# szpajder/dumphfdl

Measured on AMD Instinct MI355X. Metric: wideband I/Q Msamples/s (cf32 ingest -> decoded HFDL PDUs) at fixed channel count, higher is better.
Workload: dtype f32

## Files before the change

dumphfdl_amd/csrc/fft_kernels.hip:

```cpp
#include <hip/hip_ext.h>
#include "kernels.h"
#include "retune_launch.h"
#include "fft_core.h"
#include "fft_regs.h"

namespace hfdl {

template <int FMT>
__device__ __forceinline__ float2 load_sample(const void *__restrict__ raw, int i)
{
	if (FMT == SFMT_CS16) {
		const short2 v = ((const short2 *)raw)[i];
		return make_float2((float)v.x / 32767.5f, (float)v.y / 32767.5f);
	} else if (FMT == SFMT_CU8) {
		const uchar2 v = ((const uchar2 *)raw)[i];
		return make_float2(((float)v.x - 63.5f) / 127.0f, ((float)v.y - 63.5f) / 127.0f);
	}
	return ((const float2 *)raw)[i];
}

__device__ __forceinline__ void store_out(float2 *out, const FftOutLayout &lay, unsigned i, size_t at, float2 v)
{
	if (lay.kind == TAPL_PLAIN) { out[at] = v; return; }
	float *o = (float *)out + tap_index_f(lay.kind, 1 << lay.row_log, (size_t)(2 * lay.row_stride), lay.chan, (int)(i >> lay.row_log), (int)(i & ((1u << lay.row_log) - 1u)), 0);
	o[0] = v.x;
	o[4] = v.y;
}

template <int FMT>
__global__ __launch_bounds__(FFT_THREADS) void fft_pass1(const float2 *__restrict__ hist, FftInputs in,
		int split, float2 *__restrict__ hist_next, float2 *__restrict__ out, FftPlan p, NcoJob job, int riders)
{
	if ((int)blockIdx.x < riders) { if (blockIdx.y == 0) nco_table_segment(job, (int)blockIdx.x * FFT_THREADS + (int)threadIdx.x); return; }
	const int bid = (int)blockIdx.x - riders;
	const int rx = (int)blockIdx.y;
	const void *__restrict__ fresh = in.fresh[rx];
	if (hist != nullptr) hist += rx * in.hist_stride;
	if (hist_next != nullptr) hist_next += rx * in.hist_stride;
	out += (size_t)rx * (size_t)p.n;
	extern __shared__ float2 sm[];
	const int cs = p.n >> p.l1;
	const int c0 = bid * FFT_TILE;
	const int total = p.r1 * FFT_TILE;
	for (int e = threadIdx.x; e < total; e += FFT_THREADS) {
		const int r = e >> FFT_TILE_LOG, col = e & (FFT_TILE - 1);
		const int c = c0 + col;
		float2 v = make_float2(0.f, 0.f);
		if (c < cs) {
			const int idx = r * cs + c;
			v = idx < split ? hist[idx] : load_sample<FMT>(fresh, idx - split);
			if (hist_next != nullptr && idx >= p.n - split) hist_next[idx - (p.n - split)] = v;
		}
		sm[e] = v;
	}
	float2 *ltw = sm + total;
	for (int t = threadIdx.x; t < p.r1; t += FFT_THREADS) ltw[t] = p.tw1[t];
	__syncthreads();
	lds_fft_columns<-1>(sm, p.r1, p.l1, FFT_TILE, FFT_TILE_LOG, ltw);
	for (int e = threadIdx.x; e < total; e += FFT_THREADS) {
		const int k1 = e >> FFT_TILE_LOG, col = e & (FFT_TILE - 1);
		const int c = c0 + col;
		if (c >= cs) continue;
		float2 v = sm[bitrev(k1, p.l1) * FFT_TILE + col];
		const unsigned ex = ((unsigned)k1 * (unsigned)c) & (unsigned)(p.n - 1);
		out[(size_t)k1 * cs + c] = cmul(v, unit_twiddle(ex, p.logn));
	}
}

__global__ __launch_bounds__(FFT_THREADS) void fft_pass2(float2 *__restrict__ buf, FftPlan p, NcoJob job, int riders)
{
	if ((int)blockIdx.x < riders) { if (blockIdx.y == 0) nco_table_segment(job, (int)blockIdx.x * FFT_THREADS + (int)threadIdx.x); return; }
	const int bid = (int)blockIdx.x - riders;
	buf += (size_t)blockIdx.y * (size_t)p.n;
	extern __shared__ float2 sm[];
	const int r23 = p.n >> p.l1, ncol = p.r1 * p.r3;
	const int cc0 = bid * FFT_TILE;
	const int total = p.r2 * FFT_TILE;
	for (int e = threadIdx.x; e < total; e += FFT_THREADS) {
		const int r = e >> FFT_TILE_LOG, col = e & (FFT_TILE - 1);
		const int cc = cc0 + col;
		float2 v = make_float2(0.f, 0.f);
		if (cc < ncol) {
			const int k1 = cc >> p.l3, n3 = cc & (p.r3 - 1);
			v = buf[(size_t)k1 * r23 + (size_t)r * p.r3 + n3];
		}
// ... 169 lines not shown
			}
		}
		if (AHEAD) {
#pragma unroll
			for (int n1 = 0; n1 < 16; n1++) x[n1] = xn[n1];
		}
	}
}

template <int B>
__global__ __launch_bounds__(16 * B) void fft_rpass3(const float2 *__restrict__ in, float2 *__restrict__ out, FftPlan p, int shifted,
		FftOutLayout lay, NcoJob job, int riders, int tpw, int64_t out_rx_stride)
{
	constexpr int NT = 16 * B, R = 16 * B;
	if ((int)blockIdx.x < riders) { if (blockIdx.y == 0) nco_table_segment(job, (int)blockIdx.x * NT + (int)threadIdx.x); return; }
	in += (size_t)blockIdx.y * (size_t)p.n;
	out += blockIdx.y * out_rx_stride;
	__shared__ float2 ex[B * FR_PITCH];
	__shared__ float2 ltw[16 * B];
	const int bid = ((int)blockIdx.x - riders) * tpw, tid = (int)threadIdx.x;
	const int r23 = p.n >> p.l1;
	const int col = tid & 15, n2 = tid >> 4;
	float2 pre[16], pn[16];
	auto load = [&](float2 (&v)[16], int tile) {
		const int cc0 = tile * 16;
		const float2 *src = in + (size_t)(cc0 >> p.l1) * R + (size_t)(cc0 & (p.r1 - 1)) * r23;
#pragma unroll
		for (int i = 0; i < 16; i++) {
			const int e = tid + i * NT;
			v[i] = src[(size_t)(e / R) * r23 + (e % R)];
		}
	};
	load(pre, bid);
	ltw[tid] = p.tw3[tid];
	const unsigned half = shifted ? (unsigned)(p.n >> 1) : 0u;
	for (int t = 0; t < tpw; t++) {
		const int tile = bid + t;
		const int k2g = (tile * 16) >> p.l1, k10 = (tile * 16) & (p.r1 - 1);
		__syncthreads();
#pragma unroll
		for (int i = 0; i < 16; i++) {
			const int e = tid + i * NT, tcol = e / R, n3 = e % R;
			ex[n3 * 16 + ((tcol + n3) & 15)] = pre[i];
		}
		if (t + 1 < tpw) load(pn, tile + 1);
		__syncthreads();
		float2 x[16];
#pragma unroll
		for (int n1 = 0; n1 < 16; n1++) {
			const int r = n2 + B * n1;
			x[n1] = ex[r * 16 + ((col + r) & 15)];
		}
		__syncthreads();
		stage_a(x, ex, ltw, n2, col);
		__syncthreads();
#pragma unroll
		for (int i = 0; i < 256 / NT; i++) {
			const int tt = tid + i * NT, tcol = tt & 15, ka = tt >> 4;
			float2 z[B];
			stage_b<B>(z, ex, ka, tcol);
			const unsigned kbase = (unsigned)(k10 + tcol) + ((unsigned)k2g << p.l1);
#pragma unroll
			for (int kb = 0; kb < B; kb++) {
				const unsigned k = kbase + ((unsigned)(ka + 16 * kb) << (p.l1 + p.l2));
				const unsigned i2 = (k + half) & (unsigned)(p.n - 1);
				const size_t at = lay.row_log ? (size_t)(i2 >> lay.row_log) * (size_t)lay.row_stride + (i2 & ((1u << lay.row_log) - 1u)) : (size_t)i2;
				store_out(out, lay, i2, at, z[slot_small<B>(kb)]);
			}
		}
#pragma unroll
		for (int i = 0; i < 16; i++) pre[i] = pn[i];
	}
}

static void launch_rpass(const void *kernel, dim3 grid, int logr, hipStream_t st, hipEvent_t start, hipEvent_t stop, void **args)
{
	(void)hipExtLaunchKernel(kernel, grid, dim3(1u << logr), args, 0, st, start, stop, 0);
}
template <int B> static const void *rpass1_of(int fmt)
{
	return fmt == SFMT_CS16 ? (const void *)fft_rpass1<B, SFMT_CS16, false> : fmt == SFMT_CU8 ? (const void *)fft_rpass1<B, SFMT_CU8, false> : (const void *)fft_rpass1<B, SFMT_CF32, false>;
}

__global__ void retune_channelizer_kernel(ChanConst *cc, NcoState *chain, float2 *cont, int c, ChanConst k)
{
	if (blockIdx.x != 0 || threadIdx.x != 0) return;
	cc[c] = k;
	chain[c] = NcoState{ 0, 0.f, 0, 0 };
	cont[c] = make_float2(0.f, 0.f);
}

void launch_retune_channelizer(ChanConst *cc, NcoState *chain, float2 *cont, int c, const ChanConst &k, hipStream_t st, hipEvent_t done)
{
	hipExtLaunchKernelGGL(retune_channelizer_kernel, dim3(1), dim3(64), 0, st, nullptr, done, 0, cc, chain, cont, c, k);
}

static bool fast_plan(const FftPlan &p) { return p.l1 >= 6 && p.l1 <= 8 && p.l2 >= 6 && p.l2 <= 8 && p.l3 >= 6 && p.l3 <= 8; }

__global__ __launch_bounds__(256) void mixed_copy_kernel(float2 *__restrict__ plain, float *__restrict__ taps, const float2 *__restrict__ block,
		int dir, int l1, int l2, int l3, int q, int m, size_t rs_f, int slot)
{
	const size_t n = (size_t)1 << (l1 + l2 + l3);
	for (size_t e = (size_t)blockIdx.x * 256 + threadIdx.x; e < n; e += (size_t)gridDim.x * 256) {
		const int ka = (int)(e & 15), n3 = (int)(e >> 4) & ((1 << l3) - 1), kb = (int)(e >> (4 + l3)) & ((1 << (l2 - 4)) - 1), k1 = (int)(e >> (l2 + l3));
		const int k2 = ka + 16 * kb, jp = mixed_bin(natural_bin_of(k1, k2, q, l1), l1);
		float2 *pl = plain + ((size_t)k1 << (l2 + l3)) + ((size_t)k2 << l3) + n3;
		if (dir == 2) {
			*pl = block[((size_t)(jp >> 4) << (l2 - q + l3 + 4)) + (size_t)mixed_row(k2, n3, q, l3) * 16 + (jp & 15)];
			continue;
		}
		float *t = taps + tap_index_f(TAPL_OCTET, m, rs_f, slot, mixed_tap_row(k2, n3, q, l3), jp, 0);
		const float r3 = (float)(1 << l3), ir3 = 1.0f / r3;
		if (dir == 0) { const float2 v = *pl; t[0] = v.x * r3; t[4] = v.y * r3; }
		else *pl = make_float2(t[0] * ir3, t[4] * ir3);
	}
}

static void launch_mixed_copy(const FftPlan &p, const Geometry &g, float2 *plain, float *taps, const float2 *block, int dir, int slot, hipStream_t st)
{
	hipLaunchKernelGGL(mixed_copy_kernel, dim3(2048), dim3(256), 0, st, plain, taps, block, dir, p.l1, p.l2, p.l3, g.mix_q, g.m, (size_t)g.tap_row_stride * 2, slot);
}
void launch_mixed_tap_pack(const FftPlan &p, const Geometry &g, const float2 *plain, float2 *taps, int slot, hipStream_t st) { launch_mixed_copy(p, g, (float2 *)plain, (float *)taps, nullptr, 0, slot, st); }
void launch_mixed_tap_unpack(const FftPlan &p, const Geometry &g, const float2 *taps, int slot, float2 *plain, hipStream_t st) { launch_mixed_copy(p, g, plain, (float *)taps, nullptr, 1, slot, st); }
void launch_mixed_block_unpack(const FftPlan &p, const Geometry &g, const float2 *slot, float2 *plain, hipStream_t st) { launch_mixed_copy(p, g, plain, nullptr, slot, 2, 0, st); }

void launch_fft_forward(const FftPlan &p, const float2 *hist, const FftInputs &in, int fmt, int split, float2 *hist_next,
		float2 *work, float2 *out, bool shifted, hipStream_t st, FftOutLayout lay, hipEvent_t done, NcoJob nco, hipEvent_t input_read, hipEvent_t start, FftVariant var)
{
	const unsigned nrx = (unsigned)in.nrx;
	const int64_t ors = in.out_stride;
	const int c1 = (p.n >> p.l1), c2 = p.r1 * p.r3, c3 = p.r1 * p.r2;
	const int g1 = (c1 + FFT_TILE - 1) / FFT_TILE, g2 = (c2 + FFT_TILE - 1) / FFT_TILE, g3 = (c3 + FFT_TILE - 1) / FFT_TILE;
	nco.nseg = 3;
	if (fast_plan(p)) {
		const bool mix = var.mix_out != nullptr, run1 = var.passes & 1, run2 = var.passes & 2, run3 = var.passes & 4;
		if (mix) nco.nseg = 2;
		auto riders_of = [&](int l) { const int nt = 1 << l; return nco.cc ? (nco.nch + nt - 1) / nt : 0; };
		const int rd1 = riders_of(p.l1), rd2 = riders_of(p.l2), rd3 = mix ? 0 : riders_of(p.l3);
		auto tpw_of = [](int tiles) { return tiles % 4 == 0 && tiles >= 4096 ? 4 : tiles % 2 == 0 && tiles >= 1024 ? 2 : 1; };
		const int t3 = tpw_of(g3);
		FftPlan plan = p;
		FftInputs inputs = in;
		int tpw = 1, shift = shifted ? 1 : 0, keep = mix && run3 ? 1 : 0;
		int64_t out_stride = ors;
		nco.seg = 0;
		if (run1) {
			void *args[] = { &hist, &inputs, &split, &hist_next, &work, &plan, &nco, (void *)&rd1, &tpw };
			launch_rpass(p.l1 == 6 ? rpass1_of<4>(fmt) : p.l1 == 7 ? rpass1_of<8>(fmt) : rpass1_of<16>(fmt), dim3(g1 + rd1, nrx), p.l1, st, start, input_read, args);
		}
		nco.seg = 1;
		if (run2) {
			void *args[] = { &work, &plan, &nco, (void *)&rd2, &tpw, &var.mix_out, &var.mix_q, &keep, &var.mix_rx_stride };
			launch_rpass(p.l2 == 6 ? (const void *)fft_rpass2<4, false> : p.l2 == 7 ? (const void *)fft_rpass2<8, false> : (const void *)fft_rpass2<16, false>,
					dim3(g2 + rd2, nrx), p.l2, st, nullptr, mix || !run3 ? done : nullptr, args);
		}
		nco.seg = 2;
		if (run3) {
			void *args[] = { &work, &out, &plan, &shift, &lay, &nco, (void *)&rd3, (void *)&t3, &out_stride };
			launch_rpass(p.l3 == 6 ? (const void *)fft_rpass3<4> : p.l3 == 7 ? (const void *)fft_rpass3<8> : (const void *)fft_rpass3<16>,
					dim3(g3 / t3 + rd3, nrx), p.l3, st, nullptr, mix ? nullptr : done, args);
		}
		return;
	}
	const int riders = nco.cc ? (nco.nch + FFT_THREADS - 1) / FFT_THREADS : 0;
	const dim3 blk(FFT_THREADS);
	const size_t l1 = (size_t)p.r1 * (FFT_TILE + 1) * sizeof(float2), l2 = (size_t)p.r2 * (FFT_TILE + 1) * sizeof(float2);
	nco.seg = 0;
	if (fmt == SFMT_CS16) hipExtLaunchKernelGGL(fft_pass1<SFMT_CS16>, dim3(g1 + riders, nrx), blk, l1, st, start, input_read, 0, hist, in, split, hist_next, work, p, nco, riders);
	else if (fmt == SFMT_CU8) hipExtLaunchKernelGGL(fft_pass1<SFMT_CU8>, dim3(g1 + riders, nrx), blk, l1, st, start, input_read, 0, hist, in, split, hist_next, work, p, nco, riders);
	else hipExtLaunchKernelGGL(fft_pass1<SFMT_CF32>, dim3(g1 + riders, nrx), blk, l1, st, start, input_read, 0, hist, in, split, hist_next, work, p, nco, riders);
	nco.seg = 1;
	hipLaunchKernelGGL(fft_pass2, dim3(g2 + riders, nrx), blk, l2, st, work, p, nco, riders);
	nco.seg = 2;
	hipExtLaunchKernelGGL(fft_pass3, dim3(g3 + riders, nrx), blk, (size_t)p.r3 * (FFT_TILE + 1) * sizeof(float2), st, nullptr, done, 0,
			(const float2 *)work, out, p, shifted ? 1 : 0, lay, nco, riders, ors);
}

}
```

dumphfdl_amd/csrc/frontend.h:

```cpp
#pragma once
#include <hip/hip_runtime.h>
#include <complex>
#include <deque>
#include <memory>
#include <vector>
#include "../../include/hfdl_gpu.h"
#include "hip_handles.h"
#include "kernels.h"
#include "planner.h"
#include "retune_launch.h"
#include "launch_timers.h"
#include "demod.h"
#include "spectrum.h"
#include "export_ring.h"
#include "blanker.h"
#include "iqbal.h"
#include "notch.h"
#include "real_input.h"

namespace hfdl {

int select_device(int device);
int check_channel_span(int32_t sample_rate, int32_t nrx, int c, int32_t freq, int r, int32_t centre);
long env_long(const char *name, long lo, long hi, long otherwise);
inline int ilog2(int x) { int l = 0; while ((1 << l) < x) l++; return l; }
inline size_t sample_bytes(int fmt) { return fmt == SFMT_CS16 ? 4 : fmt == SFMT_CU8 ? 2 : 8; }
bool is_library_pinned(const void *p, size_t bytes);

struct LabConfig {
	int fold_tile = -1;
	int fold_slices = 0;
	int cu_split = 0;
	bool cu_partition = false;
	int fft_stream = -1;
	bool decode_stream = true;
	int fold_bound = -1;
	bool fold_ramp = true;
};
LabConfig read_lab_config();

struct HostFftPlan {
	FftPlan p{};
	DevBuf tw[3];
	int build(int n);
};
int upload_twiddles(int r, DevBuf &out);

int finish_stage();
struct StageFrames {
	DevBuf frames, data, scrambler;
	int upload(const float *symbols, const int32_t *modes, const int32_t *bitmask_lsb, int32_t nframes);
};


struct SpectrumHistory {
	static constexpr int CHUNK = 8;
	int rows = 0, interval = 0;
	DevBuf acc, peak;
	PinnedBuf<float> host;
	std::vector<Event> ev;
	std::vector<hfdl_gpu_spectrum_row> info;
	uint64_t open = 0;
	uint64_t open_first = 0;
	uint32_t open_blocks = 0;
	uint64_t oldest() const { const uint64_t kept = (uint64_t)rows - (open_blocks ? 1 : 0); return open > kept ? open - kept : 0; }
	void close()
	{
		info[open % (uint64_t)rows] = hfdl_gpu_spectrum_row{ open, open_first, open_blocks, 0 };
		open++;
		open_blocks = 0;
	}
};

struct SpectrumMonitor {
	int bins = 0;
	uint32_t flags = 0;
	DevBuf acc;
	DevBuf peak;
	PinnedBuf<float> host;
	DevBuf scratch;
	Event ev;
	hipEvent_t last = nullptr;
	hipEvent_t newest() const { return last ? last : ev.e; }
	uint64_t fresh = 0;
	std::vector<uint64_t> blocks, first;
	std::unique_ptr<SpectrumHistory> hist;
};

struct ChannelExport {
	int nsel = 0, format = 0;
	float scale = 1.f;
	ExportRing ring;
	DevBuf channels;
// ... 24 lines not shown
	PinnedBuf<IqbalState> host;
	Event ev;
	uint64_t step = 0;
	uint32_t seeds = 0;
};

struct Notch {
	float mu = 0.f;
	int nsel = 0;
	std::vector<bool> selected;
	DevBuf out;
	DevBuf sel;
	DevBuf state;
	DevBuf rec;
	PinnedBuf<NotchRecord> host;
	PinnedBuf<int32_t> host_sel;
	Event staged;
	bool staging = false;
	Event ev;
	bool launched = false;
};

struct Retune {
	DevBuf pad, work;
	DevBuf eo;
	PinnedBuf<float2> stage[2];
	Event staged[2];
	DoneEvent done;
	uint64_t calls = 0;
	std::vector<float> lp;
	float lp_cut = -1.f;
};

}

bool design_channel(const hfdl_gpu_frontend *fe, int rx, int32_t freq, hfdl::ChanConst &k, std::complex<float> *taps, std::vector<float> &lp, float &lp_cut);
int queue_real_taps(hfdl_gpu_frontend *fe, const float2 *host, float2 *pad, float2 *work, float2 *eo, int slot, hipStream_t st, hipEvent_t staged);

int close_boundary(hfdl_gpu_frontend *fe);
void condition_input(hfdl_gpu_frontend *fe, hfdl::FftInputs &in, int &fmt, hipStream_t st);
void launch_monitor(hfdl_gpu_frontend *fe, const float2 *spectrum, hipStream_t st);
const float2 *launch_canceller(hfdl_gpu_frontend *fe, int slot0, int nblk, hipEvent_t ready);
int canceller_retuned(hfdl_gpu_frontend *fe, int channel);
void launch_export(hfdl_gpu_frontend *fe, int slot0, int nblk);

struct hfdl_gpu_frontend {
	int device = 0;
	hfdl::Stream stream;
	hfdl::Stream stream_b;
	hfdl::Stream stream_d;
	hfdl::Stream stream_c;
	hfdl::Stream stream_f;
	bool cu_partitioned = false;
	bool own_decode_stream() const { return stream_d.owned; }
	hfdl::FftRule fft_rule = hfdl::FFT_RULE_INPUT;
	hfdl::FftOrder order;
	int side_of(bool on_device) const { return hfdl::fft_side(fft_rule, on_device); }
	hipStream_t fft_stream(int side) const { return side == hfdl::FFT_SERIAL ? stream.s : stream_f.owned ? stream_f.s : stream_c.s; }
	static constexpr int MAX_HALF = hfdl::FOLD_MAX_BLOCKS;
	static constexpr int MAX_STAGE = HFDL_GPU_PREFETCH_MAX + 1;
	static_assert(MAX_HALF == hfdl::PLAN_MAX_HALF && MAX_STAGE == hfdl::PLAN_MAX_STAGE && HFDL_GPU_FOLD_BATCH_MAX == MAX_HALF, "include/hfdl_gpu.h, kernels.h and planner.h name the same limits");

	std::deque<hfdl::DevBuf> mem;
	template <typename T> hipError_t alloc(T *&view, size_t count)
	{
		mem.emplace_back();
		const hipError_t e = mem.back().alloc(sizeof(T) * count);
		view = mem.back().as<T>();
		return e;
	}
	hfdl::HostFftPlan fft;
	hfdl::Demod demod;
	int4 *d_rx = nullptr, *d_grp = nullptr;
	float2 *d_hist[2] = { nullptr, nullptr }, *d_work = nullptr, *d_spec = nullptr, *d_taps = nullptr, *d_partial = nullptr;
	float2 *d_tw_m = nullptr;
	int n_stage = 0;
	std::unique_ptr<hfdl::DevBuf> d_stage[MAX_STAGE];
	size_t stage_cap[MAX_STAGE] = {};
	float2 *d_chan_all = nullptr;
	int *d_cnt_all = nullptr;
	hfdl::ChanConst *d_cc = nullptr;
	int2 *d_win = nullptr;
	hfdl::NcoState *d_nco = nullptr;
	hfdl::NcoState *d_nco_snap = nullptr;
	float2 *d_ph = nullptr, *d_ph_cont = nullptr;
	std::unique_ptr<hfdl::SpectrumMonitor> mon;
	float2 *monitor_scratch() const { return mon ? mon->scratch.as<float2>() : nullptr; }
	std::unique_ptr<hfdl::ChannelExport> exp;
	std::unique_ptr<hfdl::Retune> retune;
	std::unique_ptr<hfdl::Blanker> blank;
	std::unique_ptr<hfdl::Notch> notch;
	std::unique_ptr<hfdl::Iqbal> iqbal;
	hfdl::DevBuf chain_scratch;

	hfdl::DoneEvent chan[2];
	hfdl::DoneEvent fft_done;
	hfdl::DoneEvent spec[2];
	hfdl::Event ev_switch;
	hfdl::Event ev_stage_ready[MAX_STAGE];
	hfdl::Event ev_stage_free[MAX_STAGE];
	hfdl::LaunchTimers timers;
	int settle_events();

	uint64_t host_blocks = 0;
	uint64_t host_pushed = 0;
	const void *pf_ptr[MAX_STAGE] = {};
	int pf_fmt[MAX_STAGE] = {};
	hipEvent_t input_event(uint64_t host_block) const
	{
		const uint64_t newest = host_blocks - 1, span = (uint64_t)n_stage - 1;
		return ev_stage_ready[(newest - host_block <= span ? host_block : newest - span) % (uint64_t)n_stage];
	}
	int32_t sample_rate = 0, decimation = 0;
	int32_t real_rate = 0;
	std::vector<int32_t> rx_base;
	float2 *d_real = nullptr;
	size_t taps_host_len() const { return real_rate ? 2 * (size_t)plan.taps_length : (size_t)plan.taps_length; }
	float tbw = 0;
	hfdl::Plan plan{};
	hfdl::Geometry geo{};
	std::vector<int32_t> freqs;
	int nrx = 1;
	std::vector<int32_t> rx_center;
	std::vector<int32_t> rx_of;
	std::vector<hfdl::RxSpan> rx_span;
	std::vector<int4> rx_host;
	int slot_of(int c) const { return hfdl::receiver_slot(rx_span[(size_t)rx_of[(size_t)c]], c); }
	std::vector<hfdl::ChanConst> cc;
	int batch = 1;
	int fold_nb = 1;
	int half_blocks = 1;
	int half_first = 1, half_target = 1;
	int cur_half = 0, batch_fill = 0;
	int last_slot = 0;
	int last_index = 0;
	float2 *chan_slot(int slot) const { return d_chan_all + (size_t)slot * (size_t)geo.nch * (size_t)geo.outs; }
	int *cnt_slot(int slot) const { return d_cnt_all + (size_t)slot * (size_t)geo.nch; }
	int last_set = 0;
	float2 *spec_slot(int set, int i) const { return d_spec + ((size_t)set * (size_t)half_blocks + (size_t)i) * spec_stride(); }
	size_t spec_stride() const { return (size_t)nrx * (size_t)geo.n; }
	float2 *ph_slot(int set, int i) const { return d_ph + ((size_t)set * (size_t)half_blocks + (size_t)i) * ph_stride(); }
	hfdl::NcoState *snap_slot(int set, int i) const { return d_nco_snap + ((size_t)set * (size_t)half_blocks + (size_t)i) * (size_t)geo.nch; }
	size_t partial_stride() const { return (size_t)geo.nch * (size_t)geo.slices * (size_t)geo.m; }
	size_t ph_stride() const { return (size_t)geo.nch * (size_t)geo.outs; }
	double prune_tol = 0.0;
	int fold_rows_max = 0;
	bool fold_bound = false;
	uint64_t blocks = 0;
	hfdl::FftOutLayout tap_layout;
	int pending_demod_buf = -1;
	int pending_demod_nblk = 0;

	~hfdl_gpu_frontend();
};
```

dumphfdl_amd/csrc/frontend_create.cpp:

```cpp
#include <atomic>
#include <cmath>
#include <complex>
#include <cstring>
#include <thread>
#include "frontend.h"

using namespace hfdl;

extern "C" int hfdl_gpu_device_count(void)
{
	int n = 0;
	if (hipGetDeviceCount(&n) != hipSuccess) return 0;
	return n;
}

int hfdl::select_device(int device)
{
	int n = 0;
	if (hipGetDeviceCount(&n) != hipSuccess || n <= 0)
		return fail(HFDL_GPU_ENODEV, "no HIP device visible: the HFDL front end has no CPU fallback");
	if (device < 0 || device >= n) return fail(HFDL_GPU_EINVAL, "device %d out of range (%d visible)", device, n);
	HIP_TRY(hipSetDevice(device));
	hipDeviceProp_t prop;
	HIP_TRY(hipGetDeviceProperties(&prop, device));
// ... 214 lines not shown
		CREATE_TRY(fe->stream_b.create());
	}
	if (lab.decode_stream) CREATE_TRY(fe->stream_d.create());
	else fe->stream_d.alias(fe->stream_b);
	fe->demod.order.own_decode = fe->own_decode_stream();
	if (lab.fft_stream < 0 ? part.on : lab.fft_stream != 0) {
		if (part.on) CREATE_TRY(fe->stream_f.create_on_cus(part.mask_fold));
		else CREATE_TRY(fe->stream_f.create());
		fe->fft_rule = FFT_RULE_OWN;
	} else if (lab.fft_stream == 0) fe->fft_rule = FFT_RULE_SERIAL;
	CREATE_TRY(fe->stream_c.create());
	return 0;
}

static int create_frontend(hfdl_gpu_frontend *fe, int32_t nrx, const int32_t *nch_per_rx)
{
	const int nch = (int)fe->freqs.size();
	const LabConfig lab = read_lab_config();
	if (!plan_block(fe->plan, fe->tbw, fe->decimation, 0.f)) return fail(HFDL_GPU_EINVAL, "fastddc planning failed");
	const Plan &pl = fe->plan;
	Geometry &g = fe->geo;
	g.n = pl.n; g.m = pl.m; g.pre = pl.pre; g.post = pl.post; g.scrap = pl.scrap; g.post_input_size = pl.post_input_size;
	g.overlap = pl.overlap; g.input_size = pl.input_size; g.outs = (pl.post_input_size + pl.post - 1) / pl.post + 1;
	g.nch = nch;
	g.tap_layout = (pl.m % 16) == 0 && (pl.pre % 8) == 0 ? TAPL_OCTET : TAPL_PLAIN;
	g.nch_pad = plan_receiver_slots(nch_per_rx, nrx, tap_layout_group(g.tap_layout), fe->rx_span);
	for (const RxSpan &r : fe->rx_span) fe->rx_host.push_back(make_int4(r.slot0, r.slots, r.chan0, r.nch));
	g.nrx = nrx;
	g.spec_rx_stride = pl.n;
	g.rx_host = fe->rx_host.data();
	g.tap_chan_stride = pl.m; g.tap_row_stride = (int64_t)g.nch_pad * pl.m;
	g.fold_tile = lab.fold_tile;
	fe->tap_layout.kind = g.tap_layout;
	fe->tap_layout.row_log = ilog2(pl.m); fe->tap_layout.row_stride = g.tap_row_stride;
	fe->prune_tol = g.tap_layout == TAPL_OCTET && nrx == 1 && !fe->real_rate ? env_double("HFDL_GPU_FOLD_PRUNE", 1e-12, 1e-3, 0.0) : 0.0;
	fe->fold_bound = lab.fold_bound < 0 ? nch >= 128 : lab.fold_bound != 0;
	const float resamp_rate = (float)(1800 * 3) / ((float)fe->sample_rate / (float)fe->decimation);
	BatchOverrides ov;
	ov.demod_batch = (int)env_long("HFDL_GPU_DEMOD_BATCH", 1, hfdl_gpu_frontend::MAX_HALF, 0);
	ov.fold_batch = (int)env_long("HFDL_GPU_FOLD_BATCH", 1, hfdl_gpu_frontend::MAX_HALF, 0);
	ov.pruned = fe->prune_tol > 0;
	ov.fold_slices = lab.fold_slices;
	ov.no_ramp = !lab.fold_ramp;
	const BatchPlan bp = plan_batches(nch, nrx, pl.n, pl.input_size, fe->sample_rate, pl.pre, fe->fold_bound,
			[&](int want) { return Demod::fit_batch(g.outs, resamp_rate, want); }, ov);
	g.slices = bp.slices;
	g.rows_per_slice = pl.pre / g.slices;
	if (pl.m > 8192 || pl.m < 16) return fail(HFDL_GPU_ERANGE, "inverse FFT size %d unsupported", pl.m);

	if (int rc = create_streams(fe, lab)) return rc;
	for (int i = 0; i < 2; i++) {
		CREATE_TRY(fe->spec[i].own.create(EV_NO_TIMING));
		CREATE_TRY(fe->chan[i].own.create(EV_NO_TIMING));
	}
	CREATE_TRY(fe->fft_done.own.create(EV_NO_TIMING));
	CREATE_TRY(fe->ev_switch.create(EV_NO_TIMING));
	if (int rc = fe->fft.build(pl.n)) return rc;
	{
		const FftPlan &fp = fe->fft.p;
		if (!fe->real_rate && g.tap_layout == TAPL_OCTET && mixed_fold_fits(fp.l1, fp.l2, fp.l3, ilog2(pl.m), fe->prune_tol > 0) && env_long("HFDL_GPU_FOLD_SPECTRUM", 0, 1, 1) == 0) {
			g.mix_l1 = fp.l1; g.mix_q = ilog2(pl.m) - fp.l1;
			g.spec_row_stride = 16; g.spec_group_stride = 16 * (int64_t)pl.pre;
		}
	}
	const size_t n = (size_t)pl.n;
	const size_t K = (size_t)nrx;
	for (int i = 0; i < 2; i++) {
		CREATE_TRY(fe->alloc(fe->d_hist[i], (size_t)pl.overlap * K));
		CREATE_TRY(hipMemsetAsync(fe->d_hist[i], 0, sizeof(float2) * (size_t)pl.overlap * K, fe->stream));
	}
	CREATE_TRY(fe->alloc(fe->d_work, n * K));
	if (fe->real_rate) CREATE_TRY(fe->alloc(fe->d_real, n * K));
	CREATE_TRY(fe->alloc(fe->d_rx, K));
	CREATE_TRY(hipMemcpy(fe->d_rx, fe->rx_host.data(), sizeof(int4) * K, hipMemcpyHostToDevice));
	g.rx_tab = fe->d_rx;
	if (g.tap_layout == TAPL_OCTET) {
		static_assert(sizeof(FoldGroup) == sizeof(int4), "a FoldGroup entry is what the fold kernels load as an int4");
		const std::vector<FoldGroup> t = fold_group_tables(fe->rx_span, g.nch_pad / 8, FOLD_GROUP_MAX);
		CREATE_TRY(fe->alloc(fe->d_grp, t.size()));
		CREATE_TRY(hipMemcpy(fe->d_grp, t.data(), sizeof(int4) * t.size(), hipMemcpyHostToDevice));
		g.grp_tab = fe->d_grp;
	}
	CREATE_TRY(fe->alloc(fe->d_taps, n * (size_t)g.nch_pad));
	CREATE_TRY(fe->alloc(fe->d_nco, (size_t)nch));
	CREATE_TRY(hipMemsetAsync(fe->d_nco, 0, sizeof(NcoState) * (size_t)nch, fe->stream));
	CREATE_TRY(fe->alloc(fe->d_ph_cont, (size_t)nch));
	CREATE_TRY(hipMemsetAsync(fe->d_ph_cont, 0, sizeof(float2) * (size_t)nch, fe->stream));
	CREATE_TRY(fe->alloc(fe->d_cc, (size_t)nch));
	fe->mem.emplace_back();
	if (int rc = upload_twiddles(pl.m, fe->mem.back())) return rc;
	fe->d_tw_m = fe->mem.back().as<float2>();
	if (prepare_ifft_nco(pl.m) != hipSuccess)
		return fail(HFDL_GPU_EHIP, "inverse FFT of %d points: LDS attribute refused: %s", pl.m, hipGetErrorString(hipGetLastError()));
	if (int rc = build_taps(fe)) return rc;
	if (fe->prune_tol > 0 && g.tap_layout == TAPL_OCTET)
		if (int rc = build_fold_windows(fe)) return rc;
	CREATE_TRY(hipMemcpy(fe->d_cc, fe->cc.data(), sizeof(ChanConst) * (size_t)nch, hipMemcpyHostToDevice));
	fe->fold_nb = bp.fold_nb;
	if (int rc = fe->demod.init(nch, g.outs, resamp_rate, fe->freqs.data(), fe->stream, bp.batch_want)) return rc;
	fe->batch = fe->demod.batch;
	fe->half_blocks = bp.half_blocks;
	fe->half_first = fe->half_target = bp.half_first;
	fe->n_stage = bp.n_stage;
	for (int i = 0; i < fe->n_stage; i++) {
		CREATE_TRY(fe->ev_stage_ready[i].create(EV_NO_TIMING));
		CREATE_TRY(fe->ev_stage_free[i].create(EV_NO_TIMING));
	}
	const size_t hb = (size_t)fe->half_blocks;
	CREATE_TRY(fe->alloc(fe->d_spec, fe->spec_stride() * 2 * hb));
	CREATE_TRY(fe->alloc(fe->d_partial, fe->partial_stride() * hb));
	CREATE_TRY(fe->alloc(fe->d_ph, fe->ph_stride() * 2 * hb));
	CREATE_TRY(fe->alloc(fe->d_nco_snap, (size_t)nch * 2 * hb));
	CREATE_TRY(fe->alloc(fe->d_chan_all, 2 * hb * (size_t)nch * g.outs));
	CREATE_TRY(fe->alloc(fe->d_cnt_all, 2 * hb * (size_t)nch));
	CREATE_TRY(hipMemsetAsync(fe->d_cnt_all, 0, sizeof(int) * 2 * hb * (size_t)nch, fe->stream));
	CREATE_TRY(hipStreamSynchronize(fe->stream));
	return 0;
}

static int create_any(hfdl_gpu_frontend **out, int device, int32_t sample_rate, int32_t nrx, const int32_t *centerfreqs, const int32_t *freqs,
		const int32_t *nch_per_rx, int32_t real_rate, const int32_t *bases)
{
	int rc = check_create_args(out, sample_rate, nrx, centerfreqs, freqs, nch_per_rx);
	if (rc || (rc = select_device(device))) return rc;
	int32_t nch = 0;
	for (int r = 0; r < nrx; r++) nch += nch_per_rx[r];
	auto fe = std::make_unique<hfdl_gpu_frontend>();
	fe->device = device;
	fe->sample_rate = sample_rate;
	fe->decimation = fft_decimation_rate(sample_rate, 1800 * 3);
	fe->tbw = relative_transition_bw(sample_rate, 250);
	fe->freqs.assign(freqs, freqs + nch);
	fe->nrx = nrx;
	fe->rx_center.assign(centerfreqs, centerfreqs + nrx);
	fe->real_rate = real_rate;
	if (real_rate) fe->rx_base.assign(bases, bases + nrx);
	for (int r = 0; r < nrx; r++) fe->rx_of.insert(fe->rx_of.end(), (size_t)nch_per_rx[r], r);
	if ((rc = create_frontend(fe.get(), nrx, nch_per_rx))) return rc;
	*out = fe.release();
	return 0;
}

extern "C" int hfdl_gpu_frontend_create_multi(hfdl_gpu_frontend **out, int device, int32_t sample_rate, int32_t nrx,
		const int32_t *centerfreqs, const int32_t *freqs, const int32_t *nch_per_rx)
{
	return create_any(out, device, sample_rate, nrx, centerfreqs, freqs, nch_per_rx, 0, nullptr);
}

extern "C" int hfdl_gpu_frontend_create_real(hfdl_gpu_frontend **out, int device, int32_t sample_rate_real, int32_t nrx,
		const int32_t *base_freqs, const int32_t *freqs, const int32_t *nch_per_rx)
{
	if (out) *out = nullptr;
	if (!base_freqs || !freqs || !nch_per_rx || nrx < 1 || nrx > HFDL_GPU_RECEIVERS_MAX) return fail(HFDL_GPU_EINVAL, "bad arguments: null pointer, or %d receivers", nrx);
	if (sample_rate_real < REAL_RATE_MIN || (sample_rate_real & 1)) return fail(HFDL_GPU_EINVAL, "real sample rate %d: even and >= %d", sample_rate_real, REAL_RATE_MIN);
	int32_t centres[HFDL_GPU_RECEIVERS_MAX];
	for (int r = 0; r < nrx; r++) {
		if (!real_base_valid(sample_rate_real, base_freqs[r])) return fail(HFDL_GPU_EINVAL, "receiver %d: base %d Hz out of range", r, base_freqs[r]);
		centres[r] = real_equiv_centre(sample_rate_real, base_freqs[r]);
	}
	return create_any(out, device, real_equiv_rate(sample_rate_real), nrx, centres, freqs, nch_per_rx, sample_rate_real, base_freqs);
}

hfdl_gpu_frontend::~hfdl_gpu_frontend()
{
	(void)hipSetDevice(device);
	for (const hfdl::Stream *s : { &stream, &stream_b, &stream_d, &stream_c, &stream_f, &demod.st_collect }) (void)s->sync();
	if (mon) (void)hipEventSynchronize(mon->newest());
}

extern "C" void hfdl_gpu_frontend_destroy(hfdl_gpu_frontend *fe) { delete fe; }
// ... 1 lines not shown
```

dumphfdl_amd/csrc/hfdl_gpu.cpp:

```cpp
#include "frontend.h"

using namespace hfdl;


int LaunchTimers::arm(Stage s, int blocks, hipEvent_t &start, hipEvent_t &stop)
{
	if (!on) return 0;
	Timed t;
	if (!pool.empty()) {
		t = std::move(pool.back());
		pool.pop_back();
	} else {
		HIP_TRY(t.start.create(EV_TIMING));
		HIP_TRY(t.stop.create(EV_TIMING));
	}
	t.blocks = blocks;
	start = t.start;
	stop = t.stop;
	stage[s].pending.push_back(std::move(t));
	return 0;
}

int LaunchTimers::drain()
{
// ... 123 lines not shown
	*stage_idx = sb;
	return 0;
}

static int single_receiver_only(const hfdl_gpu_frontend *fe, const char *what)
{
	if (fe && fe->nrx > 1)
		return fail(HFDL_GPU_EINVAL, "%s: this front end has %d receivers -- push a block of every receiver with hfdl_gpu_frontend_push_blocks_raw()", what, fe->nrx);
	return 0;
}

extern "C" int hfdl_gpu_frontend_prefetch_block_raw(hfdl_gpu_frontend *fe, const void *raw, size_t nsamples, int sample_format)
{
	if (!fe || !raw) return fail(HFDL_GPU_EINVAL, "null argument");
	if (int rc = single_receiver_only(fe, "hfdl_gpu_frontend_prefetch_block_raw")) return rc;
	if (int rc = check_block(fe, nsamples, sample_format)) return rc;
	if (fe->host_blocks - fe->host_pushed >= (uint64_t)(fe->n_stage - 1))
		return fail(HFDL_GPU_ERANGE, "%d blocks are prefetched already (geometry.prefetch_depth): push the oldest first", fe->n_stage - 1);
	if (!is_library_pinned(raw, sample_bytes(sample_format) * nsamples)) return fail(HFDL_GPU_EINVAL, "only buffers from hfdl_gpu_host_alloc() can be prefetched");
	HIP_TRY(hipSetDevice(fe->device));
	int sb = -1;
	const void *one[1] = { raw };
	int rc = queue_input_copy(fe, one, nsamples, sample_format, &sb);
	if (rc) return rc;
	fe->pf_ptr[sb] = raw; fe->pf_fmt[sb] = sample_format;
	return 0;
}

extern "C" int hfdl_gpu_frontend_prefetch_cancel(hfdl_gpu_frontend *fe)
{
	if (!fe) return fail(HFDL_GPU_EINVAL, "null argument");
	if (int rc = single_receiver_only(fe, "hfdl_gpu_frontend_prefetch_cancel")) return rc;
	if (fe->host_pushed == fe->host_blocks) return 0;
	HIP_TRY(hipSetDevice(fe->device));
	HIP_TRY(hipEventSynchronize(fe->input_event(fe->host_blocks - 1)));
	fe->host_pushed = fe->host_blocks;
	return 0;
}


static int launch_demod(hfdl_gpu_frontend *fe, int buf, int nblk, hipEvent_t ready)
{
	const int slot0 = buf * fe->half_blocks;
	const float2 *rows = launch_canceller(fe, slot0, nblk, ready);
	if (rows) {
		HIP_TRY(hipGetLastError());
		ready = nullptr;
	} else rows = fe->chan_slot(slot0);
	return fe->demod.launch_half(rows, fe->cnt_slot(slot0), nblk, buf, ready, fe->stream_b, fe->stream_d, fe->timers);
}

static void leave_half(hfdl_gpu_frontend *fe, int nblk, bool with_demod)
{
	const int half = fe->cur_half;
	fe->last_slot = half * fe->half_blocks + nblk - 1;
	fe->last_index = nblk - 1;
	fe->cur_half ^= 1;
	if (with_demod) fe->demod.order.hand_over(half);
}

static int flush_pending_demod(hfdl_gpu_frontend *fe, bool after_fft)
{
	if (fe->pending_demod_buf < 0) return 0;
	const int buf = fe->pending_demod_buf, nblk = fe->pending_demod_nblk;
	fe->pending_demod_buf = -1;
	return launch_demod(fe, buf, nblk, after_fft ? fe->fft_done.event() : fe->chan[buf].event());
}

static int enqueue_fft(hfdl_gpu_frontend *fe, FftInputs &in, int fmt, int stage_idx, int on_device)
{
	const Geometry &g = fe->geo;
	const int i = fe->batch_fill, set = fe->cur_half;
	const FftPushPlan plan = fe->order.push(fe->side_of(on_device != 0), i, fe->half_target, fe->pending_demod_buf >= 0);
	const hipStream_t st = fe->fft_stream(plan.side);
	if (plan.flush_before)
		if (int rc = flush_pending_demod(fe, false)) return rc;
	if (plan.wait_switch) {
		HIP_TRY(hipEventRecord(fe->ev_switch, fe->fft_stream(plan.side ^ 1)));
		HIP_TRY(hipStreamWaitEvent(st, fe->ev_switch, 0));
	}
	if (plan.wait_set_free && fe->chan[set].pending()) HIP_TRY(hipStreamWaitEvent(st, fe->chan[set].event(), 0));
	if (plan.wait_first_fold) HIP_TRY(hipStreamWaitEvent(st, fe->chan[set ^ 1].event(), 0));
	if (plan.wait_retune) HIP_TRY(hipStreamWaitEvent(st, fe->retune->done.event(), 0));
	NcoJob job;
	job.cc = fe->d_cc; job.chain = fe->d_nco; job.snap = fe->snap_slot(set, i);
	job.ph = fe->ph_slot(set, i); job.cont = fe->d_ph_cont;
	job.nch = g.nch; job.outs = g.outs; job.post_input_size = g.post_input_size; job.post = g.post;
	hipEvent_t fft_start = nullptr, fft_done = nullptr;
	if (plan.side == FFT_BESIDE || plan.hold_after) {
		DoneEvent &done = plan.side == FFT_BESIDE ? fe->spec[set] : fe->fft_done;
		if (int rc = fe->timers.arm(ST_FFT, 1, done, fft_start)) return rc;
		fft_done = done.event();
	} else if (int rc = fe->timers.arm(ST_FFT, 1, fft_start, fft_done)) return rc;
	condition_input(fe, in, fmt, st);
	in.nrx = fe->nrx; in.hist_stride = g.overlap; in.out_stride = g.n;
	FftVariant var;
	float2 *spectrum = fe->spec_slot(set, i);
	if (g.mix_l1) {
		var.mix_out = spectrum; var.mix_q = g.mix_q; var.mix_rx_stride = g.n;
		spectrum = fe->monitor_scratch();
		var.passes = spectrum ? FFT_PASSES_ALL : FFT_PASSES_12;
	}
	const bool real = fe->real_rate != 0;
	launch_fft_forward(fe->fft.p, fe->d_hist[fe->blocks & 1], in, fmt, g.overlap, fe->d_hist[(fe->blocks + 1) & 1], fe->d_work, real ? fe->d_real : spectrum, !real, st,
			FftOutLayout(), real ? nullptr : fft_done, job,
			stage_idx >= 0 ? fe->ev_stage_free[stage_idx].e : nullptr,
			fft_start, var);
	if (real) {
		RealUntangleJob u;
		u.in = fe->d_real; u.out = spectrum; u.in_stride = u.out_stride = g.n; u.n = g.n; u.logn = fe->fft.p.logn; u.nrx = fe->nrx;
		launch_real_untangle(u, st, fft_done);
	}
	launch_monitor(fe, spectrum, st);
	if (plan.hold_after)
		if (int rc = flush_pending_demod(fe, true)) return rc;
	HIP_TRY(hipGetLastError());
	fe->blocks++;
	fe->batch_fill++;
	return 0;
}

static int close_half(hfdl_gpu_frontend *fe, bool launch_now, bool with_demod = true)
{
	const int nblk = fe->batch_fill;
	if (nblk == 0) return 0;
	const Geometry &g = fe->geo;
	const int half = fe->cur_half;
	const HalfClosePlan plan = fe->order.close(launch_now);
	if (plan.wait_input) HIP_TRY(hipStreamWaitEvent(fe->stream, fe->spec[half].event(), 0));
	for (int done = 0, take = 0; done < nblk; done += take) {
		take = fold_launch_blocks(g, nblk - done, fe->fold_nb);
		hipEvent_t start = nullptr, stop = nullptr;
		if (int rc = fe->timers.arm(ST_FOLD, take, start, stop)) return rc;
		if (launch_fold(g, fe->d_taps, fe->spec_slot(half, done), fe->spec_stride(), fe->d_partial + (size_t)done * fe->partial_stride(), fe->partial_stride(),
				take, fe->stream, start, stop) < 0)
			return fail(HFDL_GPU_EINVAL, "no fold launch of %d blocks on this geometry", take);
	}
	if (hipEvent_t e = fe->demod.half_read_event(half)) HIP_TRY(hipStreamWaitEvent(fe->stream, e, 0));
	if (with_demod && fe->own_decode_stream() && !fe->fold_bound) {
		if (hipEvent_t e = fe->demod.frames_free_event()) HIP_TRY(hipStreamWaitEvent(fe->stream, e, 0));
	}
	const int slot0 = half * fe->half_blocks;
	hipEvent_t ifft_start = nullptr;
	if (int rc = fe->timers.arm(ST_IFFT, nblk, fe->chan[half], ifft_start)) return rc;
	launch_ifft_nco(g, fe->d_partial, fe->partial_stride(), fe->d_cc, fe->snap_slot(half, 0), fe->ph_slot(half, 0), fe->ph_stride(), fe->d_tw_m,
			fe->chan_slot(slot0), fe->cnt_slot(slot0), nblk, fe->stream, fe->chan[half].event(), ifft_start);
	launch_export(fe, slot0, nblk);
	HIP_TRY(hipGetLastError());
	fe->last_set = half;
	fe->batch_fill = 0;
	leave_half(fe, nblk, with_demod);
	if (!with_demod) return 0;
	if (!plan.hold_back) return launch_demod(fe, half, nblk, fe->chan[half].event());
	fe->pending_demod_buf = half;
	fe->pending_demod_nblk = nblk;
	return 0;
}

int close_boundary(hfdl_gpu_frontend *fe)
{
	if (int rc = flush_pending_demod(fe, false)) return rc;
	return close_half(fe, true);
}

extern "C" int hfdl_gpu_frontend_channelize_block(hfdl_gpu_frontend *fe, const float *iq, size_t nsamples, int on_device)
{
	FftInputs in;
	int sidx = -1;
	int rc = single_receiver_only(fe, "hfdl_gpu_frontend_channelize_block");
	if (rc) return rc;
	const void *one[1] = { iq };
	int fmt = SFMT_CF32;
	if ((rc = stage_input(fe, one, nsamples, fmt, on_device, in, &sidx))) return rc;
	if ((rc = close_boundary(fe))) return rc;
	if ((rc = enqueue_fft(fe, in, SFMT_CF32, sidx, on_device))) return rc;
	return close_half(fe, false, false);
}

extern "C" int hfdl_gpu_frontend_push_baseband(hfdl_gpu_frontend *fe, const float *chan_out, const int32_t *counts)
{
	if (!fe || !chan_out || !counts) return fail(HFDL_GPU_EINVAL, "null argument");
	const Geometry &g = fe->geo;
	for (int c = 0; c < g.nch; c++)
		if (counts[c] < 0 || counts[c] > g.outs) return fail(HFDL_GPU_ERANGE, "channel %d: %d samples, a block holds at most %d", c, counts[c], g.outs);
	int rc = hfdl_gpu_frontend_sync(fe);
	if (rc) return rc;
	const int half = fe->cur_half, slot0 = half * fe->half_blocks;
	HIP_TRY(hipMemcpy(fe->chan_slot(slot0), chan_out, sizeof(float2) * (size_t)g.nch * (size_t)g.outs, hipMemcpyHostToDevice));
	HIP_TRY(hipMemcpy(fe->cnt_slot(slot0), counts, sizeof(int32_t) * (size_t)g.nch, hipMemcpyHostToDevice));
	leave_half(fe, 1, true);
	return launch_demod(fe, half, 1, nullptr);
}

static int push_any(hfdl_gpu_frontend *fe, const void *const *raw, size_t nsamples, int fmt, int on_device)
{
	FftInputs in;
	int sidx = -1;
	int rc = stage_input(fe, raw, nsamples, fmt, on_device, in, &sidx);
	if (rc) return rc;
	if ((rc = enqueue_fft(fe, in, fmt, sidx, on_device))) return rc;
	if (fe->batch_fill < fe->half_target) return 0;
	rc = close_half(fe, !fe->fold_bound);
	fe->half_target = fe->half_blocks;
	return rc;
}

extern "C" int hfdl_gpu_frontend_push_block(hfdl_gpu_frontend *fe, const float *iq, size_t nsamples, int on_device)
{
	if (int rc = single_receiver_only(fe, "hfdl_gpu_frontend_push_block")) return rc;
	const void *one[1] = { iq };
	return push_any(fe, one, nsamples, SFMT_CF32, on_device);
}

extern "C" int hfdl_gpu_frontend_push_block_raw(hfdl_gpu_frontend *fe, const void *raw, size_t nsamples, int sample_format, int on_device)
{
	if (int rc = single_receiver_only(fe, "hfdl_gpu_frontend_push_block_raw")) return rc;
	const void *one[1] = { raw };
	return push_any(fe, one, nsamples, sample_format, on_device);
}

extern "C" int hfdl_gpu_frontend_push_blocks_raw(hfdl_gpu_frontend *fe, const void *const *raw, size_t nsamples, int sample_format, int on_device)
{
	if (!fe || !raw) return fail(HFDL_GPU_EINVAL, "null argument");
	return push_any(fe, raw, nsamples, sample_format, on_device);
}


extern "C" int hfdl_gpu_frontend_retune_channel(hfdl_gpu_frontend *fe, int32_t channel, int32_t new_freq_hz)
{
	if (!fe) return fail(HFDL_GPU_EINVAL, "null argument");
	const int nch = fe->geo.nch;
	if (channel < 0 || channel >= nch) return fail(HFDL_GPU_EINVAL, "channel %d out of range (%d channels)", channel, nch);
	if (fe->prune_tol > 0) return fail(HFDL_GPU_EINVAL, "retune refused: HFDL_GPU_FOLD_PRUNE is set, and the pruned fold's row windows depend on the pass bands");
	const int rx = fe->rx_of[(size_t)channel];
	if (int rc = check_channel_span(fe->sample_rate, fe->nrx, channel, new_freq_hz, rx, fe->rx_center[(size_t)rx])) return rc;
	for (int c = 0; c < nch; c++)
		if (c != channel && fe->rx_of[(size_t)c] == rx && fe->freqs[(size_t)c] == new_freq_hz)
			return fail(HFDL_GPU_EINVAL, "channel %d of receiver %d already listens on %d Hz", c, rx, new_freq_hz);
	const size_t ntaps = fe->taps_host_len(), n = (size_t)fe->plan.n;
	ChanConst k;
	{
		std::vector<float> none;
		float cut = -1.f;
		if (!design_channel(fe, rx, new_freq_hz, k, nullptr, none, cut)) return fail(HFDL_GPU_EINVAL, "fastddc planning failed for %d channel(s)", 1);
	}
	HIP_TRY(hipSetDevice(fe->device));
	if (!fe->retune) {
		auto r = std::make_unique<Retune>();
		CREATE_TRY(r->pad.alloc(sizeof(float2) * n));
		CREATE_TRY(r->work.alloc(sizeof(float2) * n));
		if (fe->real_rate) CREATE_TRY(r->eo.alloc(sizeof(float2) * 2 * n));
		for (int i = 0; i < 2; i++) {
			CREATE_TRY(r->stage[i].alloc(ntaps));
			CREATE_TRY(r->staged[i].create(EV_NO_TIMING));
		}
		CREATE_TRY(r->done.own.create(EV_NO_TIMING));
		if (int rc = fe->demod.prepare_retune(fe->stream_b)) return rc;
		HIP_TRY(hipMemsetAsync(r->pad.p, 0, sizeof(float2) * n, fe->stream));
		fe->retune = std::move(r);
	}
	Retune &r = *fe->retune;
	const int sb = (int)(r.calls & 1);
	if (r.calls >= 2) HIP_TRY(hipEventSynchronize(r.staged[sb]));
	static_assert(sizeof(std::complex<float>) == sizeof(float2), "taps are copied as cf32");
	design_channel(fe, rx, new_freq_hz, k, (std::complex<float> *)r.stage[sb].p, r.lp, r.lp_cut);
	if (int rc = close_boundary(fe)) return rc;
	const int slot = fe->slot_of(channel);
	if (!fe->real_rate) HIP_TRY(hipMemcpyAsync(r.pad.p, r.stage[sb].p, sizeof(float2) * ntaps, hipMemcpyHostToDevice, fe->stream));
	FftOutLayout lay = fe->tap_layout;
	lay.chan = slot;
	float2 *dst = lay.kind == TAPL_PLAIN ? fe->d_taps + (size_t)slot * (size_t)fe->geo.tap_chan_stride : fe->d_taps;
	if (fe->real_rate) {
		if (int rc = queue_real_taps(fe, r.stage[sb].p, r.pad.as<float2>(), r.work.as<float2>(), r.eo.as<float2>(), slot, fe->stream, r.staged[sb])) return rc;
	} else if (fe->geo.mix_l1) {
		FftVariant v;
		v.passes = FFT_PASSES_12;
		launch_fft_forward(fe->fft.p, nullptr, r.pad.p, SFMT_CF32, 0, nullptr, r.work.as<float2>(), nullptr, true, fe->stream, FftOutLayout(), nullptr, NcoJob(), r.staged[sb], nullptr, v);
		launch_mixed_tap_pack(fe->fft.p, fe->geo, r.work.as<float2>(), fe->d_taps, slot, fe->stream);
	} else launch_fft_forward(fe->fft.p, nullptr, r.pad.p, SFMT_CF32, 0, nullptr, r.work.as<float2>(), dst, true, fe->stream, lay, nullptr, NcoJob(), r.staged[sb]);
	launch_retune_channelizer(fe->d_cc, fe->d_nco, fe->d_ph_cont, channel, k, fe->stream, r.done.signal());
	fe->demod.enqueue_retune(channel, new_freq_hz, fe->stream_b, fe->stream_d);
	if (int rc = canceller_retuned(fe, channel)) return rc;
	HIP_TRY(hipGetLastError());
	fe->order.retune();
	fe->freqs[(size_t)channel] = new_freq_hz;
	fe->cc[(size_t)channel] = k;
	r.calls++;
	return 0;
}


extern "C" int hfdl_gpu_frontend_sync(hfdl_gpu_frontend *fe)
{
	if (!fe) return fail(HFDL_GPU_EINVAL, "null argument");
	HIP_TRY(hipSetDevice(fe->device));
	if (int rc = close_boundary(fe)) return rc;
	fe->half_target = fe->half_first;
	for (const Stream *s : { &fe->stream_c, &fe->stream_f, &fe->stream, &fe->stream_b, &fe->stream_d }) HIP_TRY(s->sync());
	fe->order.drained();
	HIP_TRY(hipGetLastError());
	return fe->settle_events();
}

static int check_poll_args(const hfdl_gpu_frontend *fe, const hfdl_gpu_pdu *out, int32_t max, const int32_t *n)
{
	if (!fe || !n) return fail(HFDL_GPU_EINVAL, "null argument");
	if (!out && max > 0) return fail(HFDL_GPU_EINVAL, "null PDU buffer with max = %d", max);
	return 0;
}

extern "C" int hfdl_gpu_frontend_poll_pdus(hfdl_gpu_frontend *fe, hfdl_gpu_pdu *out, int32_t max, int32_t *n)
{
	int rc = check_poll_args(fe, out, max, n);
	if (rc || (rc = hfdl_gpu_frontend_sync(fe))) return rc;
	return fe->demod.collect(out, max, n, fe->stream_d);
}

extern "C" int hfdl_gpu_frontend_poll_pdus_ready(hfdl_gpu_frontend *fe, hfdl_gpu_pdu *out, int32_t max, int32_t *n, int32_t max_in_flight)
{
	if (max_in_flight <= 0) return hfdl_gpu_frontend_poll_pdus(fe, out, max, n);
	if (int rc = check_poll_args(fe, out, max, n)) return rc;
	*n = 0;
	HIP_TRY(hipSetDevice(fe->device));
	return fe->demod.collect_ready(max_in_flight < 2, out, max, n, fe->stream_d);
}
```

dumphfdl_amd/csrc/retune_launch.h:

```cpp
#pragma once
#include "kernels.h"

namespace hfdl {

void launch_retune_channelizer(ChanConst *cc, NcoState *chain, float2 *cont, int c, const ChanConst &k, hipStream_t st, hipEvent_t done = nullptr);

}
```

Before: 22680.

## Move NCO phasor table generation out of FFT riders into per-half kernel

NCO state advancement and phasor table writing no longer ride along inside the forward FFT passes as extra blocks. A dedicated kernel now runs once per half at close time, with one thread per channel and one grid row per block. It fills snapshots and phasor tables and double-buffers the chain state. This removes the rider blocks from the FFT launches and the continuation-phasor buffer. The cost is an extra serialized launch on the main stream, and each block row re-advances the NCO state from the start (O(nblk²) steps), which recomputes phasors by recurrence.

```diff
diff --git a/dumphfdl_amd/csrc/fft_kernels.hip b/dumphfdl_amd/csrc/fft_kernels.hip
--- a/dumphfdl_amd/csrc/fft_kernels.hip
+++ b/dumphfdl_amd/csrc/fft_kernels.hip
@@ -1,6 +1,7 @@
 #include <hip/hip_ext.h>
 #include "kernels.h"
 #include "retune_launch.h"
+#include "nco_tables.h"
 #include "fft_core.h"
 #include "fft_regs.h"
 
@@ -336,17 +337,43 @@
 	return fmt == SFMT_CS16 ? (const void *)fft_rpass1<B, SFMT_CS16, false> : fmt == SFMT_CU8 ? (const void *)fft_rpass1<B, SFMT_CU8, false> : (const void *)fft_rpass1<B, SFMT_CF32, false>;
 }
 
-__global__ void retune_channelizer_kernel(ChanConst *cc, NcoState *chain, float2 *cont, int c, ChanConst k)
+__global__ __launch_bounds__(64) void nco_tables_kernel(NcoTablesJob job)
+{
+	const int c = (int)blockIdx.x * 64 + (int)threadIdx.x, b = (int)blockIdx.y;
+	if (c >= job.nch) return;
+	const ChanConst k = job.cc[c];
+	NcoState st = job.chain[c];
+	for (int j = 0; j < b; j++) nco_advance(st, nco_output_count(st, job.post_input_size, job.post), job.post, job.post_input_size, k.nco_rate);
+	job.snap[(size_t)b * job.nch + c] = st;
+	float2 p = nco_phasor_seed(st.starting_phase);
+	float2 *dst = job.ph + (size_t)b * job.ph_stride + c;
+	const float cd = k.nco_cosdelta, sd = k.nco_sindelta;
+	const size_t row = (size_t)job.nch;
+	for (int i = 0; i < job.outs; i++, dst += row) {
+		*dst = p;
+		nco_phasor_step(p.x, p.y, cd, sd);
+	}
+	if (b == job.nblk - 1) {
+		nco_advance(st, nco_output_count(st, job.post_input_size, job.post), job.post, job.post_input_size, k.nco_rate);
+		job.chain_next[c] = st;
+	}
+}
+
+void launch_nco_tables(const NcoTablesJob &job, hipStream_t st)
+{
+	hipLaunchKernelGGL(nco_tables_kernel, dim3((job.nch + 63) / 64, job.nblk), dim3(64), 0, st, job);
+}
+
+__global__ void retune_channelizer_kernel(ChanConst *cc, NcoState *chain, int c, ChanConst k)
 {
 	if (blockIdx.x != 0 || threadIdx.x != 0) return;
 	cc[c] = k;
 	chain[c] = NcoState{ 0, 0.f, 0, 0 };
-	cont[c] = make_float2(0.f, 0.f);
-}
-
-void launch_retune_channelizer(ChanConst *cc, NcoState *chain, float2 *cont, int c, const ChanConst &k, hipStream_t st, hipEvent_t done)
-{
-	hipExtLaunchKernelGGL(retune_channelizer_kernel, dim3(1), dim3(64), 0, st, nullptr, done, 0, cc, chain, cont, c, k);
+}
+
+void launch_retune_channelizer(ChanConst *cc, NcoState *chain, int c, const ChanConst &k, hipStream_t st, hipEvent_t done)
+{
+	hipExtLaunchKernelGGL(retune_channelizer_kernel, dim3(1), dim3(64), 0, st, nullptr, done, 0, cc, chain, c, k);
 }
 
 static bool fast_plan(const FftPlan &p) { return p.l1 >= 6 && p.l1 <= 8 && p.l2 >= 6 && p.l2 <= 8 && p.l3 >= 6 && p.l3 <= 8; }
@@ -385,6 +412,7 @@
 	const int64_t ors = in.out_stride;
 	const int c1 = (p.n >> p.l1), c2 = p.r1 * p.r3, c3 = p.r1 * p.r2;
 	const int g1 = (c1 + FFT_TILE - 1) / FFT_TILE, g2 = (c2 + FFT_TILE - 1) / FFT_TILE, g3 = (c3 + FFT_TILE - 1) / FFT_TILE;
+	nco = NcoJob();
 	nco.nseg = 3;
 	if (fast_plan(p)) {
 		const bool mix = var.mix_out != nullptr, run1 = var.passes & 1, run2 = var.passes & 2, run3 = var.passes & 4;
diff --git a/dumphfdl_amd/csrc/frontend.h b/dumphfdl_amd/csrc/frontend.h
--- a/dumphfdl_amd/csrc/frontend.h
+++ b/dumphfdl_amd/csrc/frontend.h
@@ -9,6 +9,7 @@
 #include "kernels.h"
 #include "planner.h"
 #include "retune_launch.h"
+#include "nco_tables.h"
 #include "launch_timers.h"
 #include "demod.h"
 #include "spectrum.h"
@@ -199,8 +200,10 @@
 	hfdl::ChanConst *d_cc = nullptr;
 	int2 *d_win = nullptr;
 	hfdl::NcoState *d_nco = nullptr;
+	int nco_cur = 0;
+	hfdl::NcoState *nco_chain(int which) const { return d_nco + (size_t)which * (size_t)geo.nch; }
 	hfdl::NcoState *d_nco_snap = nullptr;
-	float2 *d_ph = nullptr, *d_ph_cont = nullptr;
+	float2 *d_ph = nullptr;
 	std::unique_ptr<hfdl::SpectrumMonitor> mon;
 	float2 *monitor_scratch() const { return mon ? mon->scratch.as<float2>() : nullptr; }
 	std::unique_ptr<hfdl::ChannelExport> exp;
diff --git a/dumphfdl_amd/csrc/frontend_create.cpp b/dumphfdl_amd/csrc/frontend_create.cpp
--- a/dumphfdl_amd/csrc/frontend_create.cpp
+++ b/dumphfdl_amd/csrc/frontend_create.cpp
@@ -320,10 +320,8 @@
 		g.grp_tab = fe->d_grp;
 	}
 	CREATE_TRY(fe->alloc(fe->d_taps, n * (size_t)g.nch_pad));
-	CREATE_TRY(fe->alloc(fe->d_nco, (size_t)nch));
-	CREATE_TRY(hipMemsetAsync(fe->d_nco, 0, sizeof(NcoState) * (size_t)nch, fe->stream));
-	CREATE_TRY(fe->alloc(fe->d_ph_cont, (size_t)nch));
-	CREATE_TRY(hipMemsetAsync(fe->d_ph_cont, 0, sizeof(float2) * (size_t)nch, fe->stream));
+	CREATE_TRY(fe->alloc(fe->d_nco, 2 * (size_t)nch));
+	CREATE_TRY(hipMemsetAsync(fe->d_nco, 0, sizeof(NcoState) * 2 * (size_t)nch, fe->stream));
 	CREATE_TRY(fe->alloc(fe->d_cc, (size_t)nch));
 	fe->mem.emplace_back();
 	if (int rc = upload_twiddles(pl.m, fe->mem.back())) return rc;
diff --git a/dumphfdl_amd/csrc/hfdl_gpu.cpp b/dumphfdl_amd/csrc/hfdl_gpu.cpp
--- a/dumphfdl_amd/csrc/hfdl_gpu.cpp
+++ b/dumphfdl_amd/csrc/hfdl_gpu.cpp
@@ -229,10 +229,6 @@
 	if (plan.wait_set_free && fe->chan[set].pending()) HIP_TRY(hipStreamWaitEvent(st, fe->chan[set].event(), 0));
 	if (plan.wait_first_fold) HIP_TRY(hipStreamWaitEvent(st, fe->chan[set ^ 1].event(), 0));
 	if (plan.wait_retune) HIP_TRY(hipStreamWaitEvent(st, fe->retune->done.event(), 0));
-	NcoJob job;
-	job.cc = fe->d_cc; job.chain = fe->d_nco; job.snap = fe->snap_slot(set, i);
-	job.ph = fe->ph_slot(set, i); job.cont = fe->d_ph_cont;
-	job.nch = g.nch; job.outs = g.outs; job.post_input_size = g.post_input_size; job.post = g.post;
 	hipEvent_t fft_start = nullptr, fft_done = nullptr;
 	if (plan.side == FFT_BESIDE || plan.hold_after) {
 		DoneEvent &done = plan.side == FFT_BESIDE ? fe->spec[set] : fe->fft_done;
@@ -250,7 +246,7 @@
 	}
 	const bool real = fe->real_rate != 0;
 	launch_fft_forward(fe->fft.p, fe->d_hist[fe->blocks & 1], in, fmt, g.overlap, fe->d_hist[(fe->blocks + 1) & 1], fe->d_work, real ? fe->d_real : spectrum, !real, st,
-			FftOutLayout(), real ? nullptr : fft_done, job,
+			FftOutLayout(), real ? nullptr : fft_done, NcoJob(),
 			stage_idx >= 0 ? fe->ev_stage_free[stage_idx].e : nullptr,
 			fft_start, var);
 	if (real) {
@@ -274,6 +270,14 @@
 	const Geometry &g = fe->geo;
 	const int half = fe->cur_half;
 	const HalfClosePlan plan = fe->order.close(launch_now);
+	{
+		NcoTablesJob job;
+		job.cc = fe->d_cc; job.chain = fe->nco_chain(fe->nco_cur); job.chain_next = fe->nco_chain(fe->nco_cur ^ 1);
+		job.snap = fe->snap_slot(half, 0); job.ph = fe->ph_slot(half, 0); job.ph_stride = (int64_t)fe->ph_stride();
+		job.nch = g.nch; job.nblk = nblk; job.outs = g.outs; job.post_input_size = g.post_input_size; job.post = g.post;
+		launch_nco_tables(job, fe->stream);
+		fe->nco_cur ^= 1;
+	}
 	if (plan.wait_input) HIP_TRY(hipStreamWaitEvent(fe->stream, fe->spec[half].event(), 0));
 	for (int done = 0, take = 0; done < nblk; done += take) {
 		take = fold_launch_blocks(g, nblk - done, fe->fold_nb);
@@ -425,7 +429,7 @@
 		launch_fft_forward(fe->fft.p, nullptr, r.pad.p, SFMT_CF32, 0, nullptr, r.work.as<float2>(), nullptr, true, fe->stream, FftOutLayout(), nullptr, NcoJob(), r.staged[sb], nullptr, v);
 		launch_mixed_tap_pack(fe->fft.p, fe->geo, r.work.as<float2>(), fe->d_taps, slot, fe->stream);
 	} else launch_fft_forward(fe->fft.p, nullptr, r.pad.p, SFMT_CF32, 0, nullptr, r.work.as<float2>(), dst, true, fe->stream, lay, nullptr, NcoJob(), r.staged[sb]);
-	launch_retune_channelizer(fe->d_cc, fe->d_nco, fe->d_ph_cont, channel, k, fe->stream, r.done.signal());
+	launch_retune_channelizer(fe->d_cc, fe->nco_chain(fe->nco_cur), channel, k, fe->stream, r.done.signal());
 	fe->demod.enqueue_retune(channel, new_freq_hz, fe->stream_b, fe->stream_d);
 	if (int rc = canceller_retuned(fe, channel)) return rc;
 	HIP_TRY(hipGetLastError());
diff --git a/dumphfdl_amd/csrc/nco_tables.h b/dumphfdl_amd/csrc/nco_tables.h
--- /dev/null
+++ b/dumphfdl_amd/csrc/nco_tables.h
@@ -0,0 +1,17 @@
+#pragma once
+#include "kernels.h"
+
+namespace hfdl {
+
+struct NcoTablesJob {
+	const ChanConst *cc = nullptr;
+	const NcoState *chain = nullptr;
+	NcoState *chain_next = nullptr;
+	NcoState *snap = nullptr;
+	float2 *ph = nullptr;
+	int64_t ph_stride = 0;
+	int32_t nch = 0, nblk = 0, outs = 0, post_input_size = 0, post = 0;
+};
+void launch_nco_tables(const NcoTablesJob &job, hipStream_t st);
+
+}
diff --git a/dumphfdl_amd/csrc/retune_launch.h b/dumphfdl_amd/csrc/retune_launch.h
--- a/dumphfdl_amd/csrc/retune_launch.h
+++ b/dumphfdl_amd/csrc/retune_launch.h
@@ -3,6 +3,6 @@
 
 namespace hfdl {
 
-void launch_retune_channelizer(ChanConst *cc, NcoState *chain, float2 *cont, int c, const ChanConst &k, hipStream_t st, hipEvent_t done = nullptr);
+void launch_retune_channelizer(ChanConst *cc, NcoState *chain, int c, const ChanConst &k, hipStream_t st, hipEvent_t done = nullptr);
 
 }
```

Result: no change. 22730 (median of 3 runs) (+0.2%).
